# IanYeung/RealVSR

Measured on AMD Instinct MI355X. Metric: HR frames/sec (fwd+bwd) on 5-frame 180x320 LR windows, higher is better.
Workload: dtype f32 (bf16x3 GEMM); 1 GPU; EDVR-M nf64, 5-frame 180x320 LR windows, batch 8 per GPU, x4 output, VideoSRModel.optimize_parameters: fwd + LapPyr(ssim,cb) on Y + GWLoss on CbCr + bwd + Adam step; per_gpu_batch=8, global_batch=8, parallelism=sequence-dp1, gemm=bf16x3 (3-term bf16 split on v_mfma_f32_32x32x16_bf16, f32 accumulate), lf_term=ssim (restated IQA_pytorch.SSIM, parity unpinned)

## Files before the change

### include/realvsr_hip.h

```cpp
#ifndef REALVSR_HIP_H
#define REALVSR_HIP_H
#include <stddef.h>
#ifdef __cplusplus
extern "C" {
#endif

#define RVSR_OK 0
#define RVSR_ERR_UNSUPPORTED 1
#define RVSR_ERR_BAD_ARG 2
#define RVSR_ERR_LAUNCH 3
#define RVSR_ERR_WORKSPACE 4

const char* rvsr_last_error(void);

void rvsr_set_gemm_mode(int mode);
int rvsr_get_gemm_mode(void);
void rvsr_set_gemm_mode_thread(int mode);


size_t rvsr_modulated_deform_conv_forward_workspace_bytes(int channels, int channels_out);
int rvsr_modulated_deform_conv_forward(const float* input, const float* weight, const float* bias,
                                       const float* offset, const float* mask, float* output,
                                       int batch, int channels, int height, int width, int channels_out,
                                       int kernel_h, int kernel_w, int stride_h, int stride_w,
// ... 33 lines not shown
size_t rvsr_dcn_pack_weights(const float* weight, int channels, int channels_out, void* out, size_t out_bytes,
                             long long* desc, void* stream);
int rvsr_dcn_pack_forward(const float* input, const float* weight, const float* bias, const float* om,
                          float* output, int batch, int channels, int height, int width, int channels_out,
                          int stride, int pad, int dilation, int deformable_group, int act, float slope,
                          void* probe, void* workspace, size_t workspace_bytes, void* stream);
int rvsr_dcn_pack_backward(const float* input, const float* weight, const float* om, const float* grad_output,
                           const float* act_out, float act_slope, float* grad_input, float* grad_weight,
                           float* grad_bias, float* grad_om, int batch, int channels, int height, int width,
                           int channels_out, int stride, int pad, int dilation, int deformable_group,
                           const void* probe, void* workspace, size_t workspace_bytes, void* stream);
int rvsr_dcn_pack_forward_plan(const float* input, const float* weight, const float* bias, const float* om,
                               float* output, int batch, int channels, int height, int width, int channels_out,
                               int stride, int pad, int dilation, int deformable_group, int act, float slope,
                               void* probe, void* workspace, size_t workspace_bytes, long long* plan);
int rvsr_dcn_pack_backward_plan(const float* input, const float* weight, const float* om, const float* grad_output,
                                const float* act_out, float act_slope, float* grad_input, float* grad_weight,
                                float* grad_bias, float* grad_om, int batch, int channels, int height, int width,
                                int channels_out, int stride, int pad, int dilation, int deformable_group,
                                const void* probe, void* workspace, size_t workspace_bytes, long long* plan);
int rvsr_dcn_fused_takes(int batch, int channels, int height, int width, int channels_out, int kernel_h, int kernel_w, int stride_h,
                         int stride_w, int pad_h, int pad_w, int dilation_h, int dilation_w, int group, int deformable_group);
size_t rvsr_dcn_probe_samples(int batch, int deformable_group, int height_out, int width_out);
int rvsr_dcn_forward_halo(const unsigned* counters, size_t nsamples, int channels_out);

size_t rvsr_deform_conv_generic_workspace_bytes(int dtype, int channels, int height, int width, int kernel_h, int kernel_w,
                                                int stride_h, int stride_w, int pad_h, int pad_w, int dilation_h, int dilation_w);
size_t rvsr_deform_conv_generic_forward_workspace_bytes(int dtype, int channels, int height, int width, int kernel_h, int kernel_w,
                                                        int stride_h, int stride_w, int pad_h, int pad_w, int dilation_h,
                                                        int dilation_w);
int rvsr_deform_conv_generic_forward(int dtype, const void* input, const void* weight, const void* bias, const void* offset,
                                     const void* mask, void* output, int batch, int channels, int height, int width,
                                     int channels_out, int kernel_h, int kernel_w, int stride_h, int stride_w, int pad_h, int pad_w,
                                     int dilation_h, int dilation_w, int group, int deformable_group, void* workspace,
                                     size_t workspace_bytes, void* stream);
int rvsr_deform_conv_generic_backward(int dtype, const void* input, const void* weight, const void* offset, const void* mask,
                                      const void* grad_output, void* grad_input, void* grad_offset, void* grad_mask,
                                      void* grad_weight, void* grad_bias, int batch, int channels, int height, int width,
                                      int channels_out, int kernel_h, int kernel_w, int stride_h, int stride_w, int pad_h, int pad_w,
                                      int dilation_h, int dilation_w, int group, int deformable_group, void* workspace,
                                      size_t workspace_bytes, void* stream);


size_t rvsr_conv2d_forward_workspace_bytes(int C1, int C2, int Co, int ksize);
int rvsr_conv2d_forward(const float* x1, int C1, const float* x2, int C2, const float* xact, float xact_slope,
                        int in_mode, int Hs, int Ws, const float* weight, const float* bias,
                        const float* residual, float* out1, int Co1, float* out2, int Co2, int B, int ksize,
                        int stride, int w_mode, int act, float slope, int pixel_shuffle, int Hout, int Wout,
                        void* workspace, size_t workspace_bytes, void* stream);
int rvsr_conv2d_forward_plan(const float* x1, int C1, const float* x2, int C2, const float* xact, float xact_slope,
                             int in_mode, int Hs, int Ws, const float* weight, const float* bias,
                             const float* residual, float* out1, int Co1, float* out2, int Co2, int B, int ksize,
                             int stride, int w_mode, int act, float slope, int pixel_shuffle, int Hout, int Wout, int* plan);

size_t rvsr_conv2d_pack_weights(const float* weight, int C_in, int Co, int ksize, int w_mode, void* out, size_t out_bytes,
                                long long* desc, void* stream);
int rvsr_pack_weights_batched(const void* descs, int n, void* stream);

size_t rvsr_conv2d_wgrad_workspace_bytes(int C1, int C2, int Co, int B, int ksize, int stride, int Hout, int Wout);
int rvsr_conv2d_backward_weight(const float* x1, int C1, const float* x2, int C2, int Hin, int Win,
                                const float* gout, const float* gact, float gact_slope, int g_mode,
                                int Gs_h, int Gs_w, float* grad_weight, float* grad_bias, int Co, int B,
                                int ksize, int stride, int Hout, int Wout, int accumulate,
                                void* workspace, size_t workspace_bytes, void* stream);
int rvsr_conv2d_backward_weight_plan(const float* x1, int C1, const float* x2, int C2, int Hin, int Win,
                                     const float* gout, const float* gact, float gact_slope, int g_mode,
                                     int Gs_h, int Gs_w, float* grad_weight, int Co, int B, int ksize, int stride,
                                     int Hout, int Wout, int* plan);


int rvsr_upsample_bilinear_forward(const float* in, float* out, size_t planes, int H, int W, int factor,
                                   float scale, void* stream);
int rvsr_upsample_bilinear_backward(const float* gout, float* gin, size_t planes, int H, int W, int factor,
                                    float scale, void* stream);

int rvsr_maxavgpool_forward(const float* in, float* out, unsigned char* argmax, int B, int C, int H, int W,
                            void* stream);
int rvsr_maxavgpool_backward(const float* gout, const unsigned char* argmax, float* gin, int B, int C, int H,
                             int W, void* stream);

int rvsr_tsa_temporal_forward(const float* emb, const float* emb_ref, const float* aligned, float* mod,
                              float* prob, int B, int N, int C, int H, int W, int frame_major, void* stream);
int rvsr_tsa_temporal_backward(const float* gmod, const float* emb, const float* emb_ref, const float* aligned,
                               const float* prob, float* galigned, float* gemb, float* gemb_ref, int B, int N,
                               int C, int H, int W, int frame_major, void* stream);

int rvsr_tsa_output_forward(const float* fea, const float* att, const float* att_add, float* out, size_t n,
                            void* stream);
int rvsr_tsa_output_backward(const float* g, const float* fea, const float* att, float* gfea, float* gatt,
                             size_t n, void* stream);


int rvsr_pyr_down_forward(const float* in, float* out, size_t planes, int H, int W, void* stream);
int rvsr_pyr_down_backward(const float* gout, float* gin, size_t planes, int H, int W, void* stream);
int rvsr_pyr_updiff_forward(const float* cur, const float* down, float* out, size_t planes, int H, int W,
                            void* stream);
int rvsr_pyr_updiff_backward(const float* gout, float* gdown, size_t planes, int H, int W, void* stream);

size_t rvsr_charbonnier_workspace_bytes(void);
int rvsr_charbonnier_forward(const float* x, const float* y, size_t n, float eps, double scale, float* out,
                             void* workspace, void* stream);
int rvsr_charbonnier_backward(const float* x, const float* y, const float* gscalar, float scale, float eps,
                              float* gx, size_t n, void* stream);

int rvsr_gwloss_forward(const float* x1, const float* x2, size_t planes, int H, int W, float w, double scale, float* out,
                        float* fa, float* fbx, float* fby, void* workspace, void* stream);
// ... 66 lines not shown
```

### realvsr_amd/_lib.py

```python
import ctypes
import os
import subprocess

import torch

_CSRC = os.path.join(os.path.dirname(os.path.abspath(__file__)), 'csrc')
SO_PATH = os.environ.get('RVSR_SO', os.path.join(_CSRC, 'librealvsr_hip.so'))
_lib = None

c_fp = ctypes.c_void_p
c_int, c_float, c_double, c_size = ctypes.c_int, ctypes.c_float, ctypes.c_double, ctypes.c_size_t

_CONV_CALL = [c_fp, c_int, c_fp, c_int, c_fp, c_float, c_int, c_int, c_int, c_fp, c_fp, c_fp, c_fp, c_int, c_fp, c_int, c_int, c_int,
              c_int, c_int, c_int, c_float, c_int, c_int, c_int]
SIGNATURES = {
    'rvsr_last_error': (ctypes.c_char_p, []),
    'rvsr_modulated_deform_conv_forward': (c_int, [c_fp] * 6 + [c_int] * 16 + [c_fp, c_size, c_fp]),
    'rvsr_modulated_deform_conv_forward_workspace_bytes': (c_size, [c_int] * 2),
    'rvsr_modulated_deform_conv_backward_workspace_bytes': (c_size, [c_int] * 8),
    'rvsr_modulated_deform_conv_backward': (c_int, [c_fp] * 11 + [c_int] * 16 + [c_fp, c_size, c_fp]),
    'rvsr_deform_conv_workspace_bytes': (c_size, [c_int] * 11),
    'rvsr_deform_conv_forward': (c_int, [c_fp] * 4 + [c_int] * 16 + [c_fp, c_size, c_fp]),
    'rvsr_deform_conv_backward_input': (c_int, [c_fp] * 6 + [c_int] * 16 + [c_fp, c_size, c_fp]),
    'rvsr_deform_conv_backward_parameters': (c_int, [c_fp] * 4 + [c_int] * 15 + [c_float, c_int, c_fp, c_size, c_fp]),
    'rvsr_deform_conv_generic_workspace_bytes': (c_size, [c_int] * 12),
    'rvsr_deform_conv_generic_forward_workspace_bytes': (c_size, [c_int] * 12),
    'rvsr_deform_conv_generic_forward': (c_int, [c_int] + [c_fp] * 6 + [c_int] * 15 + [c_fp, c_size, c_fp]),
    'rvsr_deform_conv_generic_backward': (c_int, [c_int] + [c_fp] * 10 + [c_int] * 15 + [c_fp, c_size, c_fp]),
    'rvsr_dcn_pack_forward': (c_int, [c_fp] * 5 + [c_int] * 10 + [c_float, c_fp, c_fp, c_size, c_fp]),
    'rvsr_dcn_offset_probe': (c_int, [c_fp, c_int, c_int, c_int, c_int, c_fp, c_fp]),
    'rvsr_dcn_pack_backward': (c_int, [c_fp] * 5 + [c_float] + [c_fp] * 4 + [c_int] * 9 + [c_fp, c_fp, c_size, c_fp]),
    'rvsr_dcn_pack_forward_plan': (c_int, [c_fp] * 5 + [c_int] * 10 + [c_float, c_fp, c_fp, c_size, ctypes.POINTER(ctypes.c_longlong)]),
    'rvsr_dcn_pack_backward_plan': (c_int, [c_fp] * 5 + [c_float] + [c_fp] * 4 + [c_int] * 9 + [c_fp, c_fp, c_size,
                                                                                             ctypes.POINTER(ctypes.c_longlong)]),
    'rvsr_dcn_fused_takes': (c_int, [c_int] * 15),
    'rvsr_dcn_probe_samples': (c_size, [c_int] * 4),
    'rvsr_dcn_forward_halo': (c_int, [c_fp, c_size, c_int]),
    'rvsr_conv2d_forward': (c_int, _CONV_CALL + [c_fp, c_size, c_fp]),
    'rvsr_conv2d_forward_plan': (c_int, _CONV_CALL + [ctypes.POINTER(c_int)]),
    'rvsr_conv2d_forward_workspace_bytes': (c_size, [c_int] * 4),
    'rvsr_conv2d_pack_weights': (c_size, [c_fp, c_int, c_int, c_int, c_int, c_fp, c_size, ctypes.POINTER(ctypes.c_longlong), c_fp]),
    'rvsr_dcn_pack_weights': (c_size, [c_fp, c_int, c_int, c_fp, c_size, ctypes.POINTER(ctypes.c_longlong), c_fp]),
    'rvsr_pack_weights_batched': (c_int, [c_fp, c_int, c_fp]),
    'rvsr_set_gemm_mode': (None, [c_int]),
    'rvsr_get_gemm_mode': (c_int, []),
    'rvsr_set_gemm_mode_thread': (None, [c_int]),
    'rvsr_conv2d_wgrad_workspace_bytes': (c_size, [c_int] * 8),
    'rvsr_conv2d_backward_weight': (c_int, [c_fp, c_int, c_fp, c_int, c_int, c_int, c_fp, c_fp, c_float, c_int, c_int,
                                            c_int, c_fp, c_fp, c_int, c_int, c_int, c_int, c_int, c_int, c_int, c_fp,
                                            c_size, c_fp]),
    'rvsr_conv2d_backward_weight_plan': (c_int, [c_fp, c_int, c_fp, c_int, c_int, c_int, c_fp, c_fp, c_float, c_int, c_int, c_int, c_fp] +
                                         [c_int] * 6 + [ctypes.POINTER(c_int)]),
    'rvsr_upsample_bilinear_forward': (c_int, [c_fp, c_fp, c_size, c_int, c_int, c_int, c_float, c_fp]),
    'rvsr_upsample_bilinear_backward': (c_int, [c_fp, c_fp, c_size, c_int, c_int, c_int, c_float, c_fp]),
    'rvsr_maxavgpool_forward': (c_int, [c_fp, c_fp, c_fp, c_int, c_int, c_int, c_int, c_fp]),
    'rvsr_maxavgpool_backward': (c_int, [c_fp, c_fp, c_fp, c_int, c_int, c_int, c_int, c_fp]),
    'rvsr_tsa_temporal_forward': (c_int, [c_fp] * 5 + [c_int] * 6 + [c_fp]),
    'rvsr_tsa_temporal_backward': (c_int, [c_fp] * 8 + [c_int] * 6 + [c_fp]),
    'rvsr_tsa_output_forward': (c_int, [c_fp] * 4 + [c_size, c_fp]),
    'rvsr_tsa_output_backward': (c_int, [c_fp] * 5 + [c_size, c_fp]),
    'rvsr_pyr_down_forward': (c_int, [c_fp, c_fp, c_size, c_int, c_int, c_fp]),
    'rvsr_pyr_down_backward': (c_int, [c_fp, c_fp, c_size, c_int, c_int, c_fp]),
    'rvsr_pyr_updiff_forward': (c_int, [c_fp, c_fp, c_fp, c_size, c_int, c_int, c_fp]),
    'rvsr_pyr_updiff_backward': (c_int, [c_fp, c_fp, c_size, c_int, c_int, c_fp]),
    'rvsr_charbonnier_workspace_bytes': (c_size, []),
    'rvsr_charbonnier_forward': (c_int, [c_fp, c_fp, c_size, c_float, c_double, c_fp, c_fp, c_fp]),
    'rvsr_charbonnier_backward': (c_int, [c_fp, c_fp, c_fp, c_float, c_float, c_fp, c_size, c_fp]),
    'rvsr_gwloss_forward': (c_int, [c_fp, c_fp, c_size, c_int, c_int, c_float, c_double, c_fp, c_fp, c_fp, c_fp, c_fp, c_fp]),
    'rvsr_gwloss_backward': (c_int, [c_fp, c_fp, c_fp, c_fp, c_float, c_fp, c_size, c_int, c_int, c_fp]),
    'rvsr_ycbcr_to_bgr_u8': (c_int, [c_fp, c_fp, c_int, c_int, c_fp]),
    'rvsr_reduce_workspace_bytes': (c_size, []),
    'rvsr_pixel_loss_forward': (c_int, [c_fp, c_fp, c_size, c_int, c_float, c_double, c_fp, c_fp, c_fp]),
    'rvsr_pixel_loss_backward': (c_int, [c_fp, c_fp, c_fp, c_int, c_float, c_float, c_fp, c_size, c_fp]),
    'rvsr_ssim_forward': (c_int, [c_fp, c_fp, c_size, c_int, c_int, c_double, c_fp, c_fp, c_fp, c_fp, c_fp, c_fp]),
    'rvsr_ssim_backward': (c_int, [c_fp] * 6 + [c_float, c_fp, c_size, c_int, c_int, c_fp]),
    'rvsr_conv_gauss_forward': (c_int, [c_fp, c_fp, c_size, c_int, c_int, c_float, c_fp]),
    'rvsr_conv_gauss_backward': (c_int, [c_fp, c_fp, c_size, c_int, c_int, c_float, c_fp]),
    'rvsr_pyr_upsample_forward': (c_int, [c_fp, c_fp, c_size, c_int, c_int, c_fp]),
    'rvsr_pyr_upsample_backward': (c_int, [c_fp, c_fp, c_size, c_int, c_int, c_fp]),
    'rvsr_adam_step': (c_int, [c_fp] * 4 + [c_size] + [c_float] * 6 + [c_fp]),
    'rvsr_bcast_add_act': (c_int, [c_fp, c_fp, c_size, c_int, c_int, c_float, c_fp]),
    'rvsr_bcast_reduce_act': (c_int, [c_fp, c_fp, c_fp, c_size, c_int, c_float, c_fp]),
    'rvsr_augment_clips': (c_int, [c_fp] * 5 + [c_size] + [c_int] * 10 + [c_float, c_fp]),
    'rvsr_bn_workspace_bytes': (c_size, [c_int] * 3),
    'rvsr_bn_lrelu_forward': (c_int, [c_fp] * 9 + [c_int] * 4 + [c_float] * 3 + [c_fp, c_size, c_fp]),
    'rvsr_bn_lrelu_backward': (c_int, [c_fp] * 9 + [c_int] * 4 + [c_float, c_fp, c_size, c_fp]),
    'rvsr_gan_loss_forward': (c_int, [c_fp, c_size, c_fp, c_size, c_float, c_double, c_fp, c_fp, c_fp]),
    'rvsr_gan_loss_backward': (c_int, [c_fp, c_size, c_size, c_fp, c_fp, c_float, c_float, c_fp, c_fp, c_fp]),
    'rvsr_channel_attention_workspace_bytes': (c_size, [c_int] * 4),
    'rvsr_channel_attention_plan': (c_int, [c_int] * 4 + [c_fp] * 3 + [ctypes.POINTER(c_int)] * 2),
    'rvsr_channel_attention_forward': (c_int, [c_fp] * 10 + [c_int] * 5 + [c_float, c_fp, c_size, c_fp]),
    'rvsr_channel_attention_backward': (c_int, [c_fp] * 12 + [c_int] * 5 + [c_float, c_fp, c_size, c_fp]),
# ... 74 lines not shown
```

### realvsr_amd/csrc/conv2_kernels.hip

```cpp
#define RVSR_DEFINE_PACK
#include "conv_plan.h"

#include "bf16x3.h"

#ifdef RVSR_ABL5
constexpr int ABL5 = RVSR_ABL5;
#else
constexpr int ABL5 = 0;
#endif

#ifdef RVSR_TIMELINE
__device__ unsigned long long rvsr_dbg[512];
extern "C" int rvsr_debug_read(unsigned long long* out) { return (int)hipMemcpyFromSymbol(out, HIP_SYMBOL(rvsr_dbg), sizeof(unsigned long long) * 512); }
#define STAMP(i) do { if (blockIdx.x == 77 && tid == 0) rvsr_dbg[(i)] = __builtin_amdgcn_s_memtime(); } while (0)
#else
#define STAMP(i) do {} while (0)
#endif

template <int MT, int MODE>
__device__ __forceinline__ void conv2_epilogue(f32x16 (&acc)[MT][2], const ConvFwdParams& p, const float* bias_s, int b,
                                               int o0, int row0, int col, int hi) {
    const float neg = p.act == 0 ? 1.f : (p.act == 1 ? 0.f : p.slope);
    const bool col_ok = col < p.Wout;
    const size_t HW = (size_t)p.Hout * p.Wout;
#pragma unroll
    for (int n = 0; n < 2; ++n) {
        const int row = row0 + n;
        if (row >= p.Hout) continue;
        const size_t pix = (size_t)row * p.Wout + col;
#pragma unroll
        for (int m = 0; m < MT; ++m) {
            float resv[16];
            if (MODE == 1) {
#pragma unroll
                for (int r = 0; r < 16; ++r) {
                    const int o = o0 + m * 32 + 4 * hi + (r & 3) + 8 * (r >> 2);
                    const bool ok = col_ok && o < p.Co;
                    resv[r] = p.res[ok ? ((size_t)b * p.Co + o) * HW + pix : 0];
                }
            }
#pragma unroll
            for (int r = 0; r < 16; ++r) {
                const int ol = m * 32 + 4 * hi + (r & 3) + 8 * (r >> 2);
                const int o = o0 + ol;
                const bool ok = col_ok && o < p.Co;
                const int oc = ok ? o : 0;
                float v = acc[m][n][r] + bias_s[ol];
                v = v > 0.f ? v : v * neg;
                if (MODE == 3) {
                    const size_t idx = (((size_t)b * (p.Co >> 2) + (oc >> 2)) * (2 * p.Hout) + 2 * row + ((oc >> 1) & 1)) *
                                           (2 * p.Wout) + 2 * col + (oc & 1);
                    if (ok) p.out1[idx] = v;
                } else if (MODE == 2) {
                    const bool first = oc < p.Co1;
                    float* dst = first ? p.out1 : p.out2;
                    const size_t idx = ((size_t)b * (first ? p.Co1 : p.Co - p.Co1) + (first ? oc : oc - p.Co1)) * HW + pix;
// ... 294 lines not shown
#pragma unroll
                for (int g = 0; g < CCG; ++g) {
                    const int oc = 2 * g + hi;
                    bf16x8 ah[MT], al[MT], bh[2], bl[2];
#pragma unroll
                    for (int m = 0; m < MT; ++m) {
                        ah[m] = ws_hi[(tap * NOCT + oc) * MP + m * 32 + lo];
                        al[m] = ws_lo[(tap * NOCT + oc) * MP + m * 32 + lo];
                    }
#pragma unroll
                    for (int n = 0; n < 2; ++n) {
                        const int idx = (oc * IH + (wave * 2 + n) * STRIDE + dy) * IW + lo * STRIDE + dx;
                        bh[n] = xs_hi[idx];
                        bl[n] = xs_lo[idx];
                    }
#pragma unroll
                    for (int m = 0; m < MT; ++m)
#pragma unroll
                        for (int n = 0; n < 2; ++n) acc[m][n] = mfma_bf16(ah[m], bh[n], acc[m][n]);
#pragma unroll
                    for (int m = 0; m < MT; ++m)
#pragma unroll
                        for (int n = 0; n < 2; ++n) acc[m][n] = mfma_bf16(ah[m], bl[n], acc[m][n]);
#pragma unroll
                    for (int m = 0; m < MT; ++m)
#pragma unroll
                        for (int n = 0; n < 2; ++n) acc[m][n] = mfma_bf16(al[m], bh[n], acc[m][n]);
                }
            }
            STAMP(4 + chunk * 5);
            __syncthreads();
            STAMP(5 + chunk * 5);
        }
        if (p.ps)
            conv2_epilogue<MT, 3>(acc, p, bias_s, cb_, cmb * MP, cy0 + wave * 2, cx0 + lo, hi);
        else if (p.out2 != nullptr)
            conv2_epilogue<MT, 2>(acc, p, bias_s, cb_, cmb * MP, cy0 + wave * 2, cx0 + lo, hi);
        else if (p.res != nullptr) {
            if (p.vec4) conv2_epilogue_v4<MT, 1>(acc, p, bias_s, cb_, cmb * MP, cy0 + wave * 2, cx0, lo, hi);
            else conv2_epilogue<MT, 1>(acc, p, bias_s, cb_, cmb * MP, cy0 + wave * 2, cx0 + lo, hi);
        } else {
            if (p.vec4) conv2_epilogue_v4<MT, 0>(acc, p, bias_s, cb_, cmb * MP, cy0 + wave * 2, cx0, lo, hi);
            else conv2_epilogue<MT, 0>(acc, p, bias_s, cb_, cmb * MP, cy0 + wave * 2, cx0 + lo, hi);
        }
        STAMP(30);
        if (S + nwq < range1) {
            decode(S + nwq);
            tile_views();
            if (PF) issue_loads(0);
        }
        STAMP(31);
        __syncthreads();
    }
}

template <int MT, bool ACT_IN, int VEC, bool WIDE = false, int NT = 3>
__global__ __launch_bounds__(512, 2) void conv_fwd5_kernel(const ConvFwdParams p) {
    constexpr int KS = 3, T = 9, PAD = 1, NW = 8, TH = WIDE ? NW : 2 * NW, TW = WIDE ? 64 : 32, NTHR = NW * 64;
    constexpr int IH = TH + KS - 1, IW = TW + KS - 1;
    constexpr int MP = MT * 32, NOCT = 2, NPOS = IH * IW, NX = NOCT * NPOS;
    constexpr int WVEC = T * NOCT * MP;
    extern __shared__ __attribute__((aligned(16))) unsigned char smem_raw[];
    bf16x8* xs_base = reinterpret_cast<bf16x8*>(smem_raw);
    bf16x8* ws_base = xs_base + 2 * 2 * NX;
    float* bias_base = reinterpret_cast<float*>(ws_base + 2 * 2 * WVEC);
    bf16x8* const sink = reinterpret_cast<bf16x8*>(bias_base + 4 * MP);
    const int tid = threadIdx.x, lane = tid & 63, wave = tid >> 6, lo = lane & 31, hi = lane >> 5;
    const TView& va = p.in.a;
    const TView& vb = p.in.b;
    const int C1 = va.C, Ctot = va.C + vb.C;
    const int nchunks = (Ctot + 15) / 16;

    const unsigned nmb = (p.Co + MP - 1) / MP, nty = (p.Hout + TH - 1) / TH, ntx = (p.Wout + TW - 1) / TW;
    const unsigned items = ntx * nty * nmb * p.B;
    const unsigned xcd = blockIdx.x & 7, wq = blockIdx.x >> 3, nwq = (gridDim.x + 7 - xcd) >> 3;
    const unsigned q8 = items >> 3, r8 = items & 7;
    const unsigned range0 = xcd < r8 ? xcd * (q8 + 1) : r8 * (q8 + 1) + (xcd - r8) * q8;
    const unsigned range1 = range0 + q8 + (xcd < r8 ? 1 : 0);
    const unsigned S0 = range0 + wq;
    if (S0 >= range1) return;
    const int ntile = (int)((range1 - S0 + nwq - 1) / nwq);
    const int Q = ntile * nchunks;

    struct Tile { int x0, y0, mb, b; };
    auto tile_of = [&](int k) {
        const unsigned S = S0 + (unsigned)k * nwq;
        Tile t;
        const unsigned u = S % (ntx * nty);
        t.x0 = (int)(u % ntx) * TW;
        t.y0 = (int)(u / ntx) * TH;
        t.mb = (int)((S / (ntx * nty)) % nmb);
        t.b = (int)(S / (ntx * nty * nmb));
        return t;
    };

    constexpr int NG = TW / 4 + 2;
    __amdgpu_buffer_rsrc_t w_rs = buf_view_2g(p.wpack), xa_rs = buf_view_2g(va.p), xb_rs = buf_view_2g(va.p), act_rs = buf_view_2g(va.p);
    constexpr int NIT = VEC ? 1 : (NX + NTHR - 1) / NTHR;
    constexpr int WPARTS = NT >= 3 ? 2 : 1;
    constexpr int NWV = (WPARTS * WVEC + NTHR - 1) / NTHR;
    constexpr int NV = VEC ? 4 : 1;
    int it_oc[NIT], it_sp[NIT], it_dst[NIT];
    bool it_pos_ok[NIT];
    auto item_geom = [&](const Tile& t) {
#pragma unroll
        for (int i = 0; i < NIT; ++i) {
// ... 408 lines not shown
#define ROW(KS, STRIDE, MT, CCG) \
    if (ksize == KS && stride == STRIDE && q.mt == MT) return q.act_in ? conv_fwd2_kernel<KS, STRIDE, MT, CCG, true, 4> : conv_fwd2_kernel<KS, STRIDE, MT, CCG, false, 4>
    ROW(3, 2, 1, 1);
    ROW(3, 2, 2, 1);
    ROW(5, 1, 1, 1);
    ROW(5, 2, 1, 1);
    ROW(1, 1, 1, 2);
    ROW(1, 1, 2, 2);
#undef ROW
    return nullptr;
}

static ConvFwdKernel fwd5_kernel(const ConvFwdPlan& q) {
#define ROW(MT, VEC, WIDE, NT) \
    if (q.mt == MT && q.vec == VEC && q.wide == WIDE && q.nt == NT) return q.act_in ? conv_fwd5_kernel<MT, true, VEC, WIDE, NT> : conv_fwd5_kernel<MT, false, VEC, WIDE, NT>
    ROW(2, 1, true, 3);
    ROW(2, 1, true, 2);
    ROW(2, 1, true, 1);
    ROW(2, 1, false, 3);
    ROW(2, 1, false, 2);
    ROW(2, 1, false, 1);
    ROW(2, 2, false, 3);
    ROW(2, 2, false, 2);
    ROW(2, 2, false, 1);
    ROW(2, 3, false, 3);
    ROW(2, 3, false, 2);
    ROW(2, 3, false, 1);
    ROW(2, 0, false, 3);
    ROW(1, 0, false, 3);
    ROW(1, 1, false, 3);
    ROW(1, 2, false, 3);
    ROW(1, 3, false, 3);
#undef ROW
    if (q.mt == 2 && q.vec == 1 && q.nt == 4 && !q.act_in) return q.wide ? conv_fwd5_kernel<2, false, 1, true, 4> : conv_fwd5_kernel<2, false, 1, false, 4>;
    return nullptr;
}

int rvsr_launch_conv_fwd2(ConvFwdParams p, const ConvFwdPlan& q, int ksize, int stride, void* workspace, size_t workspace_bytes, hipStream_t st) {
    const int Ctot = p.in.a.C + p.in.b.C, T = ksize * ksize;
    int mt, ccg, nchunks, nmb;
    conv_fwd2_geom(ksize, p.Co, Ctot, mt, ccg, nchunks, nmb);
    const size_t need = rvsr_conv_fwd2_workspace_bytes(ksize, p.Co, Ctot);
    if (!workspace || workspace_bytes < need) FAIL(RVSR_ERR_WORKSPACE, "conv2d: workspace %zu B < %zu B", workspace_bytes, need);
    const bool five = q.family == CONV_FWD5;
    const ConvFwdKernel k = five ? fwd5_kernel(q) : fwd2_kernel(ksize, stride, q);
    if (!k) FAIL(RVSR_ERR_LAUNCH, "conv2d: no %s instantiation for this plan", five ? "conv_fwd5" : "conv_fwd2");
    if (!p.prepacked) {
        const size_t total = (size_t)nmb * nchunks * T * (2 * ccg) * (mt * 32);
        hipLaunchKernelGGL(pack_weights_kernel, dim3((unsigned)((total + 255) / 256)), dim3(256), 0, st, p.w, (bf16x8*)workspace, p.Co,
                           Ctot, T, mt * 32, ccg, nchunks, nmb, p.w_mode | (p.fmt ? 0x100 : 0));
    }
    p.wpack = workspace;
    p.vec4 = q.vec4;
    return rvsr_conv_launch(five ? "conv_fwd5" : "conv_fwd2", k, dim3(q.gx), five ? 512 : 256, q.lds, st, p);
}

extern "C" size_t rvsr_conv2d_pack_weights(const float* weight, int C_in, int Co, int ksize, int w_mode, void* out, size_t out_bytes,
                                           long long* desc, void* stream) {
    int mt, ccg, nchunks, nmb;
    if (ksize != 1 && ksize != 3 && ksize != 5) return 0;
    conv_fwd2_geom(ksize, Co, C_in, mt, ccg, nchunks, nmb);
    const size_t need = rvsr_conv_fwd2_workspace_bytes(ksize, Co, C_in);
    if (!weight || !out || out_bytes < need) return 0;
    if ((w_mode & 4) && !conv_f16fp8_ok(ksize, 1, mt, w_mode & 1)) return 0;
    const int fmtflag = (w_mode & 4) ? 0x100 : 0;
    const int T = ksize * ksize;
    const size_t total = (size_t)nmb * nchunks * T * (2 * ccg) * (mt * 32);
    hipLaunchKernelGGL(pack_weights_kernel, dim3((unsigned)((total + 255) / 256)), dim3(256), 0, (hipStream_t)stream, weight, (bf16x8*)out, Co,
                       C_in, T, mt * 32, ccg, nchunks, nmb, (w_mode & 1) | fmtflag);
    if (desc) {
        desc[0] = (long long)(uintptr_t)weight; desc[1] = (long long)(uintptr_t)out;
        desc[2] = Co; desc[3] = C_in; desc[4] = T; desc[5] = mt * 32; desc[6] = ccg; desc[7] = nchunks; desc[8] = nmb; desc[9] = (w_mode & 1) | fmtflag;
    }
    return need;
}
extern "C" int rvsr_pack_weights_batched(const void* descs, int n, void* stream) {
    if (n <= 0) return RVSR_OK;
    if (!descs) FAIL(RVSR_ERR_BAD_ARG, "pack_weights_batched: null table");
    static_assert(sizeof(PackDesc) == 48, "PackDesc layout is part of the C ABI (two pointers + eight ints)");
    hipLaunchKernelGGL(pack_weights_batched_kernel, dim3(16, (unsigned)n), dim3(256), 0, (hipStream_t)stream, (const PackDesc*)descs);
    hipError_t e = hipGetLastError();
    if (e != hipSuccess) FAIL(RVSR_ERR_LAUNCH, "pack_weights_batched launch: %s", hipGetErrorString(e));
    return RVSR_OK;
}

#define WG2_THREADS 512
#define WG2_GP 272
#define WG2_XP 496

typedef unsigned int u32x4 __attribute__((ext_vector_type(4)));

__device__ __forceinline__ bf16x8 as_bf16x8(u32x4 v) { return __builtin_bit_cast(bf16x8, v); }

template <int SHIFT>
__device__ __forceinline__ bf16x8 take8(u32x4 a, u32x4 b) {
    u32x4 r;
    if (SHIFT == 4) {
        r[0] = a[2]; r[1] = a[3]; r[2] = b[0]; r[3] = b[1];
    } else if (SHIFT == 3) {
        r[0] = __builtin_amdgcn_alignbit(a[2], a[1], 16);
        r[1] = __builtin_amdgcn_alignbit(a[3], a[2], 16);
        r[2] = __builtin_amdgcn_alignbit(b[0], a[3], 16);
        r[3] = __builtin_amdgcn_alignbit(b[1], b[0], 16);
    } else {
        r[0] = __builtin_amdgcn_alignbit(a[3], a[2], 16);
        r[1] = __builtin_amdgcn_alignbit(b[0], a[3], 16);
// ... 761 lines not shown
```

### realvsr_amd/csrc/conv_kernels.hip

```cpp
#include "rvsr_common.h"

#include "conv_plan.h"

template <int KS, int STRIDE, int MT, int CC>
__global__ __launch_bounds__(RVSR_WG, 2) void conv_fwd_kernel(const ConvFwdParams p) {
    constexpr int T = KS * KS, PAD = KS / 2, TH = 8, TW = 32;
    constexpr int IH = (TH - 1) * STRIDE + KS, IW = (TW - 1) * STRIDE + KS;
    constexpr int MP = MT * 32, MPP = MP + 1;
    extern __shared__ __attribute__((aligned(16))) float smem[];
    float* xs = smem;
    float* ws = smem + CC * IH * IW;
    const int tid = threadIdx.x, lane = tid & 63, wave = tid >> 6, lo = lane & 31, hi = lane >> 5;
    const int tx = blockIdx.x % p.ntx, ty = blockIdx.x / p.ntx;
    const int x0 = tx * TW, y0 = ty * TH, mb = blockIdx.y, b = blockIdx.z;
    const int Ctot = p.in.a.C + p.in.b.C;

    f32x16 acc[MT][2];
#pragma unroll
    for (int m = 0; m < MT; ++m) {
        acc[m][0] = zero16();
        acc[m][1] = zero16();
    }

    for (int c0 = 0; c0 < Ctot; c0 += CC) {
// ... 281 lines not shown
    p.Co = Co1 + Co2;
    if (pixel_shuffle && (p.Co % 4)) FAIL(RVSR_ERR_BAD_ARG, "conv2d: pixel-shuffle needs Co %% 4 == 0");
    p.B = B;
    p.Hout = Hout;
    p.Wout = Wout;
    p.w_mode = w_mode & 1;
    p.prepacked = (w_mode >> 1) & 1;
    p.fmt = (w_mode >> 2) & 1;
    p.act = act;
    p.slope = slope;
    p.ps = pixel_shuffle;
    p.ntx = (Wout + 31) / 32;
    return RVSR_OK;
}
static int conv_fwd_refuse(const ConvFwdPlan& q) {
    snprintf(rvsr_g_err, sizeof(rvsr_g_err), "%s", q.msg ? q.msg : "");
    return q.rc;
}

extern "C" int rvsr_conv2d_forward(const float* x1, int C1, const float* x2, int C2, const float* xact,
                                   float xact_slope, int in_mode, int Hs, int Ws, const float* weight,
                                   const float* bias, const float* residual, float* out1, int Co1, float* out2,
                                   int Co2, int B, int ksize, int stride, int w_mode, int act, float slope,
                                   int pixel_shuffle, int Hout, int Wout, void* workspace, size_t workspace_bytes,
                                   void* stream) {
    ConvFwdParams p;
    const int rc = conv_fwd_params(p, x1, C1, x2, C2, xact, xact_slope, in_mode, Hs, Ws, weight, bias, residual, out1, Co1, out2, Co2, B,
                                   ksize, stride, w_mode, act, slope, pixel_shuffle, Hout, Wout);
    if (rc) return rc;
    const ConvFwdPlan q = conv_fwd_plan(p, ksize, stride, rvsr_gemm_mode_now());
    if (q.rc) return conv_fwd_refuse(q);
    hipStream_t st = (hipStream_t)stream;
    switch (q.family) {
        case CONV_FWD_THIN: return rvsr_launch_conv_fwd_thin(p, q, st);
        case CONV_FWD_F32: return launch_fwd(p, q, ksize, stride, st);
        default: return rvsr_launch_conv_fwd2(p, q, ksize, stride, workspace, workspace_bytes, st);
    }
}
extern "C" int rvsr_conv2d_forward_plan(const float* x1, int C1, const float* x2, int C2, const float* xact,
                                        float xact_slope, int in_mode, int Hs, int Ws, const float* weight,
                                        const float* bias, const float* residual, float* out1, int Co1, float* out2,
                                        int Co2, int B, int ksize, int stride, int w_mode, int act, float slope,
                                        int pixel_shuffle, int Hout, int Wout, int* plan) {
    ConvFwdParams p;
    const int rc = conv_fwd_params(p, x1, C1, x2, C2, xact, xact_slope, in_mode, Hs, Ws, weight, bias, residual, out1, Co1, out2, Co2, B,
                                   ksize, stride, w_mode, act, slope, pixel_shuffle, Hout, Wout);
    if (rc) return rc;
    const ConvFwdPlan q = conv_fwd_plan(p, ksize, stride, rvsr_gemm_mode_now());
    const int row[14] = {q.family, q.mt, q.vec, q.wide, q.nt, q.act_in, q.cc, q.vec4, q.th, q.tw, (int)q.gx, (int)q.gy, (int)q.gz, (int)q.lds};
    for (int i = 0; plan && i < 14; ++i) plan[i] = row[i];
    return q.rc ? conv_fwd_refuse(q) : RVSR_OK;
}

int rvsr_g_gemm_mode = 0;
thread_local int rvsr_t_gemm_mode = -1;
extern "C" void rvsr_set_gemm_mode(int mode) { rvsr_g_gemm_mode = (mode >= 0 && mode <= 3) ? mode : 0; }
extern "C" void rvsr_set_gemm_mode_thread(int mode) { rvsr_t_gemm_mode = (mode >= 0 && mode <= 3) ? mode : -1; }
extern "C" int rvsr_get_gemm_mode() { return rvsr_gemm_mode_now(); }
extern "C" size_t rvsr_conv2d_forward_workspace_bytes(int C1, int C2, int Co, int ksize) {
    return rvsr_conv_fwd2_workspace_bytes(ksize, Co, C1 + C2);
}

extern "C" size_t rvsr_conv2d_wgrad_workspace_bytes(int C1, int C2, int Co, int B, int ksize, int stride, int Hout,
                                                    int Wout) {
    const size_t P = conv_wgrad_max_P(ksize, stride, B, Hout, Wout, Co, C1 + C2);
    return sizeof(float) * P * ((size_t)Co * (C1 + C2) * ksize * ksize + Co);
}

template <int KS, int STRIDE, int CCW>
static int launch_wgrad(const ConvWgradParams& p, int gy, int gz, hipStream_t st) {
    constexpr int IH = 3 * STRIDE + KS, IW = 31 * STRIDE + KS, CS = (IH * IW) | 1;
    return rvsr_conv_launch("conv_wgrad", conv_wgrad_kernel<KS, STRIDE, CCW>, dim3(p.P, gy, gz), RVSR_WG, sizeof(float) * (128 * 65 + CCW * CS), st, p);
}

static int conv_wgrad_params(ConvWgradParams& p, const float* x1, int C1, const float* x2, int C2, int Hin, int Win, const float* gout,
                             const float* gact, float gact_slope, int g_mode, int Gs_h, int Gs_w, float* grad_weight, int Co, int B,
                             int ksize, int stride, int Hout, int Wout) {
    if (!x1 || !gout || !grad_weight || B <= 0) FAIL(RVSR_ERR_BAD_ARG, "conv2d_backward_weight: null/empty argument");
    if ((x2 == nullptr) != (C2 == 0)) FAIL(RVSR_ERR_BAD_ARG, "conv2d_backward_weight: x2/C2 disagree");
    if (ksize != 1 && ksize != 3 && ksize != 5) FAIL(RVSR_ERR_UNSUPPORTED, "conv2d_backward_weight: kernel size %d", ksize);
    if (stride != 1 && !(stride == 2 && ksize != 1)) FAIL(RVSR_ERR_UNSUPPORTED, "conv2d_backward_weight: stride %d", stride);
    if (g_mode != 0 && g_mode != 2) FAIL(RVSR_ERR_UNSUPPORTED, "conv2d_backward_weight: gradient view mode %d", g_mode);
    make_view(p.x.a, x1, nullptr, 0.f, C1, Hin, Win, 0, 0, 0);
    make_view(p.x.b, x2, nullptr, 0.f, C2, Hin, Win, 0, 0, 0);
    if (make_view(p.g, gout, gact, gact_slope, Co, Gs_h, Gs_w, g_mode, 0, 0) || p.g.Hv != Hout || p.g.Wv != Wout)
        FAIL(RVSR_ERR_BAD_ARG, "conv2d_backward_weight: gradient view %dx%d (mode %d) vs output %dx%d", Gs_h, Gs_w, g_mode,
             Hout, Wout);
    const int pad = ksize / 2;
    if ((Hin + 2 * pad - ksize) / stride + 1 != Hout || (Win + 2 * pad - ksize) / stride + 1 != Wout)
        FAIL(RVSR_ERR_BAD_ARG, "conv2d_backward_weight: input %dx%d does not give output %dx%d", Hin, Win, Hout, Wout);
    p.part = p.bpart = nullptr;
    p.B = B;
    p.Co = Co;
    p.Hout = Hout;
    p.Wout = Wout;
    p.ntx = (Wout + 31) / 32;
    p.nty = (Hout + 3) / 4;
    p.P = 0;
    p.ring = 0;
    return RVSR_OK;
}

extern "C" int rvsr_conv2d_backward_weight_plan(const float* x1, int C1, const float* x2, int C2, int Hin, int Win,
                                                const float* gout, const float* gact, float gact_slope, int g_mode,
                                                int Gs_h, int Gs_w, float* grad_weight, int Co, int B, int ksize, int stride,
                                                int Hout, int Wout, int* plan) {
// ... 48 lines not shown
```

### realvsr_amd/csrc/conv_plan.h

```cpp
#pragma once
#include "conv_common.h"

static inline bool conv_al16(const void* a, const void* b = nullptr, const void* c = nullptr, const void* d = nullptr) {
    return ((((uintptr_t)a) | ((uintptr_t)b) | ((uintptr_t)c) | ((uintptr_t)d)) & 15) == 0;
}
static inline bool conv_span_ok(size_t H, size_t W, size_t C) { return sizeof(float) * H * W * C < ((size_t)1 << 31); }


enum ConvFwdFamily {
    CONV_FWD_THIN = 0,
    CONV_FWD5 = 1,
    CONV_FWD2 = 2,
    CONV_FWD_F32 = 3,
};

struct ConvFwdPlan {
    int rc;
    const char* msg;
    int family;
    int mt;
    int vec;
    int wide;
    int nt;
    int act_in;
    int cc;
    int vec4;
    int th, tw;
    unsigned gx, gy, gz;
    size_t lds;
};

static inline void conv_fwd2_geom(int ksize, int Co, int Ctot, int& mt, int& ccg, int& nchunks, int& nmb) {
    mt = (Co <= 32 || ksize == 5) ? 1 : 2;
    ccg = ksize == 1 ? 2 : 1;
    nchunks = (Ctot + 16 * ccg - 1) / (16 * ccg);
    nmb = (Co + mt * 32 - 1) / (mt * 32);
}
static inline bool conv_f16fp8_ok(int ksize, int stride, int mt, int w_mode) { return ksize == 3 && stride == 1 && mt == 2 && w_mode == 0; }

#define THIN_FW 136
#define THIN_FPL (10 * THIN_FW)
static inline bool conv_fwd_thin_ok(const ConvFwdParams& p, int ksize, int stride) {
    const TView& va = p.in.a;
    return ksize == 3 && stride == 1 && p.Co <= 4 && p.in.b.C == 0 && va.C % 8 == 0 && va.mode == 0 && va.act == nullptr &&
           p.out2 == nullptr && !p.ps && p.w_mode == 0 && p.Wout % 4 == 0 && va.Ws == p.Wout && va.Hs == p.Hout &&
           conv_al16(va.p, p.out1, p.res) && conv_span_ok(p.Hout, p.Wout, va.C) && va.C <= 256;
}

static inline ConvFwdPlan conv_fwd_refusal(const char* msg) {
    ConvFwdPlan r = {};
    r.rc = RVSR_ERR_UNSUPPORTED;
    r.msg = msg;
    r.family = -1;
    return r;
}

static inline ConvFwdPlan conv_fwd_plan(const ConvFwdParams& p, int ksize, int stride, int gemm_mode) {
    const TView& va = p.in.a;
    const TView& vb = p.in.b;
    const int Ctot = va.C + vb.C, T = ksize * ksize;
    if (p.act == 3 && (!p.res || ksize != 3 || stride != 1 || p.ps || p.out2 || gemm_mode == 1)) return conv_fwd_refusal(nullptr);
    ConvFwdPlan q = {};
    q.act_in = va.act != nullptr;
    q.nt = 3;
    q.th = 8;
    q.tw = 32;
    int ccg, nchunks, nmb;
    conv_fwd2_geom(ksize, p.Co, Ctot, q.mt, ccg, nchunks, nmb);
    const int ntx = (p.Wout + 31) / 32, nty8 = (p.Hout + 7) / 8;

    bool split = p.act == 3;
    const bool thin = !split && conv_fwd_thin_ok(p, ksize, stride);
    if (!split && !thin) {
        split = gemm_mode != 1 && (va.mode != 1 || ksize == 3) && (vb.C == 0 || va.C % 8 == 0);
        if (split && (ksize != 3 || stride == 2) && va.mode == 0 &&
            (!conv_span_ok(va.Hs, va.Ws, va.C > vb.C ? va.C : vb.C) || (vb.C != 0 && va.C % (16 * ccg) != 0)))
            split = false;
    }
    if (p.fmt && !(split && conv_f16fp8_ok(ksize, stride, q.mt, p.w_mode)))
        return conv_fwd_refusal("conv2d: the f16 + fp8 format (w_mode | 4) is for forward 3x3 / stride-1 convs with more than 32 output channels");

    if (thin) {
        q.family = CONV_FWD_THIN;
        q.mt = 1;
        q.tw = 128;
        q.gx = (unsigned)p.B * nty8 * ((p.Wout + 127) / 128);
        q.gy = q.gz = 1;
        q.lds = sizeof(float) * (8 * THIN_FPL + (size_t)va.C * 36);
        return q;
    }
    if (!split) {
        q.family = CONV_FWD_F32;
        q.mt = p.Co <= 32 ? 1 : (p.Co <= 64 ? 2 : 4);
        const int wide_m = q.mt == 4;
        q.cc = ksize == 1 ? 32 : ksize == 3 ? (stride == 1 ? (wide_m ? 8 : 16) : (wide_m ? 4 : 8)) : (stride == 1 ? (wide_m ? 4 : 8) : 4);
        const int IH = 7 * stride + ksize, IW = 31 * stride + ksize;
        q.lds = sizeof(float) * ((size_t)q.cc * IH * IW + (size_t)T * q.cc * (q.mt * 32 + 1));
        q.gx = (unsigned)(ntx * nty8);
        q.gy = (unsigned)((p.Co + q.mt * 32 - 1) / (q.mt * 32));
        q.gz = (unsigned)p.B;
        return q;
    }
    q.vec4 = (p.Wout % 4 == 0) && conv_al16(p.out1, p.res) && !p.ps && p.out2 == nullptr && conv_span_ok(p.Hout, p.Wout, p.Co);
    q.cc = ccg;
    q.gy = q.gz = 1;
    long items = (long)nmb * p.B;
    if (ksize != 3 || stride != 1) {
        q.family = CONV_FWD2;
        const int IH = 7 * stride + ksize, IW = 31 * stride + ksize;
        q.lds = (size_t)16 * (2 * (2 * ccg) * IH * IW + 2 * T * (2 * ccg) * (q.mt * 32)) + sizeof(float) * q.mt * 32;
        items *= (long)ntx * nty8;
        const int slots = 256 * (q.lds > 80 * 1024 ? 1 : 2);
        q.gx = (unsigned)(items < slots ? items : slots);
        return q;
    }
    q.family = CONV_FWD5;
    const bool al = conv_al16(va.p, va.act, vb.p);
    if (va.mode == 0 && va.Ws % 4 == 0 && va.Wv == va.Ws && al && conv_span_ok(va.Hs, va.Ws, va.C > vb.C ? va.C : vb.C) &&
        (vb.C == 0 || va.C % 16 == 0))
        q.vec = 1;
    else if (va.mode == 2 && vb.C == 0 && va.C % 16 == 0 && va.Wv % 4 == 0 && va.Ws == 2 * va.Wv && va.Hs == 2 * va.Hv && al &&
             conv_span_ok(va.Hs, va.Ws, va.C >> 2))
        q.vec = 2;
    else if (va.mode == 1 && vb.C == 0 && va.Wv % 4 == 0 && va.Wv == 2 * va.Ws && va.Hv <= 2 * va.Hs && va.Ws % 2 == 0 && al &&
             conv_span_ok(va.Hs, va.Ws, va.C))
        q.vec = 3;
    if (p.fmt && (q.vec != 1 || q.act_in))
        return conv_fwd_refusal("conv2d: the f16 + fp8 format needs a plain 16-byte-aligned input view with W % 4 == 0 and no act' tensor");
    const long px_n = (long)((p.Hout + 15) / 16 * 16) * ((p.Wout + 31) / 32 * 32), px_w = (long)((p.Hout + 7) / 8 * 8) * ((p.Wout + 63) / 64 * 64);
    q.wide = q.mt == 2 && q.vec == 1 && q.vec4 && px_w <= px_n;
    if (p.act == 3 && !q.wide) return conv_fwd_refusal(nullptr);
    if (p.fmt) q.nt = 4;
    else if (q.mt == 2 && q.vec != 0) q.nt = gemm_mode == 2 ? 2 : (gemm_mode == 3 ? 1 : 3);
    q.th = q.wide ? 8 : 16;
    q.tw = q.wide ? 64 : 32;
    const int NX = q.wide ? 2 * 10 * 66 : 2 * 18 * 34, WVEC = 9 * 2 * q.mt * 32;
    q.lds = (size_t)16 * (2 * 2 * NX + 2 * 2 * WVEC) + sizeof(float) * 4 * q.mt * 32 + 16;
    items *= (long)((p.Wout + q.tw - 1) / q.tw) * ((p.Hout + q.th - 1) / q.th);
    q.gx = (unsigned)(items < 256 ? items : 256);
    return q;
}

enum ConvWgradFamily {
    CONV_WGRAD_THIN = 0,
    CONV_WGRAD2,
    CONV_WGRAD5,
    CONV_WGRAD_F32_5,
    CONV_WGRAD_1X1S,
    CONV_WGRAD_1X1,
    CONV_WGRAD_F32_3S1,
    CONV_WGRAD_S2,
    CONV_WGRAD_F32_3S2,
    CONV_WGRAD_F32_1,
    CONV_WGRAD_FAMILIES
};
struct ConvWgradPlan {
    int family, P, gy, gz;
};

static inline bool conv_wgrad_can(int family, int ksize, int stride, int Co) {
    switch (family) {
        case CONV_WGRAD_THIN: return ksize == 3 && stride == 1 && Co <= 4;
        case CONV_WGRAD2: case CONV_WGRAD_F32_3S1: return ksize == 3 && stride == 1;
        case CONV_WGRAD5: case CONV_WGRAD_F32_5: return ksize == 5;
        case CONV_WGRAD_S2: case CONV_WGRAD_F32_3S2: return ksize == 3 && stride == 2;
        default: return ksize == 1;
// ... 79 lines not shown
```

Before: 83.78 HR frames/s.

## Add streaming persistent 1x1 conv forward kernel with XCD-aware tile scheduling

Adds a new persistent kernel for 1x1 stride-1 convolutions. It runs one workgroup per CU, and the work is split into contiguous ranges per XCD. Each block streams 512-pixel tiles through double-buffered LDS with register prefetch, holds activations resident across output-channel blocks when there are two input chunks, and fuses bias, activation and residual into a vectorized epilogue. It is meant to beat the generic conv_fwd2 path on large 1x1 layers by overlapping global loads with bf16x3 MFMA work. The cost is a new, complex kernel with its own occupancy and scheduling assumptions, plus a variant query API.

New measurement: 84.16 HR frames/s (median of 6 runs). No clear change (+0.4%).

```diff
diff --git a/include/realvsr_hip.h b/include/realvsr_hip.h
--- a/include/realvsr_hip.h
+++ b/include/realvsr_hip.h
@@ -109,6 +109,10 @@
                              int in_mode, int Hs, int Ws, const float* weight, const float* bias,
                              const float* residual, float* out1, int Co1, float* out2, int Co2, int B, int ksize,
                              int stride, int w_mode, int act, float slope, int pixel_shuffle, int Hout, int Wout, int* plan);
+int rvsr_conv2d_forward_variant(const float* x1, int C1, const float* x2, int C2, const float* xact, float xact_slope,
+                                int in_mode, int Hs, int Ws, const float* weight, const float* bias,
+                                const float* residual, float* out1, int Co1, float* out2, int Co2, int B, int ksize,
+                                int stride, int w_mode, int act, float slope, int pixel_shuffle, int Hout, int Wout, int* variant);
 
 size_t rvsr_conv2d_pack_weights(const float* weight, int C_in, int Co, int ksize, int w_mode, void* out, size_t out_bytes,
                                 long long* desc, void* stream);
diff --git a/realvsr_amd/_lib.py b/realvsr_amd/_lib.py
--- a/realvsr_amd/_lib.py
+++ b/realvsr_amd/_lib.py
@@ -38,6 +38,7 @@
     'rvsr_dcn_forward_halo': (c_int, [c_fp, c_size, c_int]),
     'rvsr_conv2d_forward': (c_int, _CONV_CALL + [c_fp, c_size, c_fp]),
     'rvsr_conv2d_forward_plan': (c_int, _CONV_CALL + [ctypes.POINTER(c_int)]),
+    'rvsr_conv2d_forward_variant': (c_int, _CONV_CALL + [ctypes.POINTER(c_int)]),
     'rvsr_conv2d_forward_workspace_bytes': (c_size, [c_int] * 4),
     'rvsr_conv2d_pack_weights': (c_size, [c_fp, c_int, c_int, c_int, c_int, c_fp, c_size, ctypes.POINTER(ctypes.c_longlong), c_fp]),
     'rvsr_dcn_pack_weights': (c_size, [c_fp, c_int, c_int, c_fp, c_size, ctypes.POINTER(ctypes.c_longlong), c_fp]),
diff --git a/realvsr_amd/csrc/conv2_kernels.hip b/realvsr_amd/csrc/conv2_kernels.hip
--- a/realvsr_amd/csrc/conv2_kernels.hip
+++ b/realvsr_amd/csrc/conv2_kernels.hip
@@ -2,6 +2,7 @@
 #include "conv_plan.h"
 
 #include "bf16x3.h"
+#include <type_traits>
 
 #ifdef RVSR_ABL5
 constexpr int ABL5 = RVSR_ABL5;
@@ -402,6 +403,229 @@
         STAMP(31);
         __syncthreads();
     }
+}
+
+template <int MODE>
+__device__ __forceinline__ void conv2s_epilogue(f32x16 (&acc)[2][2], const ConvFwdParams& p, const float* bias_s, int b, int o0, int pxw,
+                                                int lo, int hi) {
+    const float neg = p.act == 0 ? 1.f : (p.act == 1 ? 0.f : p.slope);
+    const int j = lo & 3;
+    const unsigned HW = (unsigned)(p.Hout * p.Wout), HW4 = 4u * HW;
+    const __amdgpu_buffer_rsrc_t out_rs = buf_view_2g(p.out1 + (size_t)b * p.Co * HW);
+    const __amdgpu_buffer_rsrc_t res_rs = buf_view_2g(MODE == 1 ? p.res + (size_t)b * p.Co * HW : p.out1);
+#pragma unroll
+    for (int n = 0; n < 2; ++n) {
+        const unsigned px = (unsigned)(pxw + 32 * n + (lo & ~3));
+        const bool px_ok = px < HW;
+        const unsigned lane_off = 4u * ((unsigned)(4 * hi + j) * HW + px);
+#pragma unroll
+        for (int m = 0; m < 2; ++m) {
+#pragma unroll
+            for (int rp = 0; rp < 4; rp += 2) {
+                float4 resv[2];
+                unsigned off[2];
+#pragma unroll
+                for (int r2 = 0; r2 < 2; ++r2) {
+                    const int ob = o0 + m * 32 + 8 * (rp + r2);
+                    off[r2] = (px_ok && ob + 4 * hi + j < p.Co ? lane_off : 0x80000000u) + (ob < p.Co ? (unsigned)ob * HW4 : 0u);
+                    if (MODE == 1) {
+                        typedef float f32x4v __attribute__((ext_vector_type(4)));
+                        const f32x4v q = __builtin_bit_cast(f32x4v, __builtin_amdgcn_raw_buffer_load_b128(res_rs, (int)off[r2], 0, 0));
+                        resv[r2] = make_float4(q.x, q.y, q.z, q.w);
+                    }
+                }
+#pragma unroll
+                for (int r2 = 0; r2 < 2; ++r2) {
+                    const int rg = rp + r2;
+                    float r0 = acc[m][n][4 * rg + 0], r1 = acc[m][n][4 * rg + 1], r2_ = acc[m][n][4 * rg + 2], r3 = acc[m][n][4 * rg + 3];
+                    quad_transpose4(r0, r1, r2_, r3, lo);
+                    const float bb = bias_s[m * 32 + 8 * rg + 4 * hi + j];
+                    float4 v = make_float4(r0 + bb, r1 + bb, r2_ + bb, r3 + bb);
+                    v.x = v.x > 0.f ? v.x : v.x * neg; v.y = v.y > 0.f ? v.y : v.y * neg;
+                    v.z = v.z > 0.f ? v.z : v.z * neg; v.w = v.w > 0.f ? v.w : v.w * neg;
+                    if (MODE == 1) { v.x += resv[r2].x; v.y += resv[r2].y; v.z += resv[r2].z; v.w += resv[r2].w; }
+                    buf_store4(out_rs, off[r2], 0u, v);
+                }
+            }
+        }
+    }
+}
+
+template <bool ACT_IN, bool RESIDENT>
+__global__ __launch_bounds__(F2S_THREADS, 1) void conv_fwd2s_kernel(const ConvFwdParams p) {
+    constexpr int XROW = F2S_XROW, XBUF = 2 * 4 * XROW, WBUF = 2 * 4 * 64;
+    constexpr unsigned OOB = 0x80000000u;
+    extern __shared__ __attribute__((aligned(16))) unsigned char smem_raw[];
+    bf16x8* xs = reinterpret_cast<bf16x8*>(smem_raw);
+    bf16x8* ws = xs + 2 * XBUF;
+    float* bias_s = reinterpret_cast<float*>(ws + 2 * WBUF);
+    const int tid = threadIdx.x, lane = tid & 63, wave = tid >> 6, lo = lane & 31, hi = lane >> 5;
+    const TView& va = p.in.a;
+    const TView& vb = p.in.b;
+    const int C1 = va.C, Ctot = va.C + vb.C;
+    const int nchunks = (Ctot + 31) / 32, nmb = (p.Co + 63) / 64;
+    const int HW = p.Hout * p.Wout;
+    const unsigned hw4 = 4u * (unsigned)HW;
+    const unsigned tpi = (unsigned)(HW + F2S_TP - 1) / F2S_TP;
+
+    const unsigned items = tpi * p.B;
+    const unsigned xcd = blockIdx.x & 7, wq = blockIdx.x >> 3, nwq = (gridDim.x + 7 - xcd) >> 3;
+    const unsigned q8 = items >> 3, r8 = items & 7;
+    const unsigned range0 = xcd < r8 ? xcd * (q8 + 1) : r8 * (q8 + 1) + (xcd - r8) * q8;
+    const unsigned range1 = range0 + q8 + (xcd < r8 ? 1 : 0);
+    const unsigned S0 = range0 + wq;
+    if (S0 >= range1) return;
+    const int ntile = (int)((range1 - S0 + nwq - 1) / nwq);
+    constexpr bool resident = RESIDENT;
+    const int Q = ntile * nmb * nchunks;
+
+    for (int i = tid; i < nmb * 64; i += F2S_THREADS) bias_s[i] = (p.bias != nullptr && i < p.Co) ? p.bias[i] : 0.f;
+
+    typedef float f32x4v __attribute__((ext_vector_type(4)));
+    f32x4v xr[2][8];
+    f32x4v ar[ACT_IN ? 8 : 1];
+    bf16x8 wr[2];
+    const int ocx = __builtin_amdgcn_readfirstlane(tid >> 7), gx4 = tid & 127;
+    const __amdgpu_buffer_rsrc_t w_rs = buf_view_2g(p.wpack);
+
+    struct Cursor { int k, c, m; };
+    Cursor xcur = {0, 0, 0}, acur = {0, 0, 0};
+    int wm = 0, wc = 0;
+    auto advance = [&](Cursor& u) {
+        if (++u.c == nchunks) {
+            u.c = 0;
+            if (resident || ++u.m == nmb) { u.m = 0; ++u.k; }
+        }
+    };
+    auto issue8 = [&](const Cursor& u, f32x4v (&dst)[8], bool act) {
+        const bool valid = u.k < ntile;
+        const unsigned S = valid ? S0 + (unsigned)u.k * nwq : S0;
+        const unsigned b = S / tpi, t0 = (S - b * tpi) * (F2S_TP / 4);
+        const int c0 = u.c * 32;
+        const bool second = c0 >= C1;
+        const int Cb = second ? vb.C : va.C, cl0 = (second ? c0 - C1 : c0) + 8 * ocx;
+        const __amdgpu_buffer_rsrc_t rs = buf_view_2g((act ? va.act : (second ? vb.p : va.p)) + (size_t)b * Cb * HW);
+        const unsigned quad = t0 + (unsigned)gx4;
+        const unsigned vo = valid && 4u * quad < (unsigned)HW ? 16u * quad : OOB;
+#pragma unroll
+        for (int j = 0; j < 8; ++j) {
+            const unsigned vo_j = cl0 + j < Cb ? vo : OOB;
+            const unsigned so = (unsigned)(cl0 + j) * hw4;
+            dst[j] = __builtin_bit_cast(f32x4v, __builtin_amdgcn_raw_buffer_load_b128(rs, (int)vo_j, (int)so, 0));
+        }
+    };
+    auto issue_x = [&](auto par) {
+        constexpr int PAR = decltype(par)::value;
+        issue8(xcur, xr[PAR], false);
+        advance(xcur);
+    };
+    auto issue_a = [&]() {
+        if (ACT_IN) {
+            issue8(acur, reinterpret_cast<f32x4v (&)[8]>(ar), true);
+            advance(acur);
+        }
+    };
+    auto issue_w = [&](auto par) {
+        constexpr int PAR = decltype(par)::value;
+        const unsigned so = (unsigned)(wm * nchunks + wc) * (WBUF * 16u);
+        wr[PAR] = __builtin_bit_cast(bf16x8, __builtin_amdgcn_raw_buffer_load_b128(w_rs, tid * 16, (int)so, 0));
+        if (++wc == nchunks) {
+            wc = 0;
+            if (++wm == nmb) wm = 0;
+        }
+    };
+    auto commit_x = [&](auto par) {
+        constexpr int PAR = decltype(par)::value;
+        bf16x8* dst = xs + PAR * XBUF + ocx * XROW + gx4;
+#pragma unroll
+        for (int e = 0; e < 4; ++e) {
+            float v[8];
+#pragma unroll
+            for (int j = 0; j < 8; ++j) v[j] = ACT_IN ? xr[PAR][j][e] * (ar[ACT_IN ? j : 0][e] > 0.f ? 1.f : va.slope) : xr[PAR][j][e];
+            bf16x8 h8, l8;
+            split8(v, h8, l8);
+            dst[e * 132] = h8;
+            dst[4 * XROW + e * 132] = l8;
+        }
+    };
+
+    f32x16 acc[2][2];
+    int ck = 0, cm = 0, cc = 0;
+    unsigned cb_ = S0 / tpi, cpx0 = (S0 - cb_ * tpi) * F2S_TP;
+    auto step = [&](auto par) {
+        constexpr int PAR = decltype(par)::value;
+        const bool xload = !resident || cm == 0;
+        if (xload) commit_x(par);
+        ws[PAR * WBUF + tid] = wr[PAR];
+        __syncthreads();
+        issue_w(par);
+        __builtin_amdgcn_sched_barrier(0);
+        if (xload) {
+            issue_a();
+            issue_x(par);
+        }
+        __builtin_amdgcn_sched_barrier(0);
+        if (cc == 0) {
+#pragma unroll
+            for (int m = 0; m < 2; ++m) {
+                acc[m][0] = zero16();
+                acc[m][1] = zero16();
+            }
+        }
+        const bf16x8* xb = xs + PAR * XBUF;
+        const bf16x8* wb = ws + PAR * WBUF;
+#pragma unroll
+        for (int g = 0; g < 2; ++g) {
+            const int oc = 2 * g + hi;
+            bf16x8 ah[2], al[2];
+#pragma unroll
+            for (int m = 0; m < 2; ++m) {
+                ah[m] = wb[oc * 64 + m * 32 + lo];
+                al[m] = wb[4 * 64 + oc * 64 + m * 32 + lo];
+            }
+#pragma unroll
+            for (int n = 0; n < 2; ++n) {
+                const int idx = oc * XROW + (lo & 3) * 132 + ((wave * 64 + n * 32 + lo) >> 2);
+                const bf16x8 bh = xb[idx], bl = xb[4 * XROW + idx];
+#pragma unroll
+                for (int m = 0; m < 2; ++m) acc[m][n] = mfma_bf16(ah[m], bh, acc[m][n]);
+#pragma unroll
+                for (int m = 0; m < 2; ++m) acc[m][n] = mfma_bf16(ah[m], bl, acc[m][n]);
+#pragma unroll
+                for (int m = 0; m < 2; ++m) acc[m][n] = mfma_bf16(al[m], bh, acc[m][n]);
+            }
+        }
+        if (++cc == nchunks) {
+            cc = 0;
+            if (p.res != nullptr) conv2s_epilogue<1>(acc, p, bias_s + cm * 64, (int)cb_, cm * 64, (int)cpx0 + wave * 64, lo, hi);
+            else conv2s_epilogue<0>(acc, p, bias_s + cm * 64, (int)cb_, cm * 64, (int)cpx0 + wave * 64, lo, hi);
+            if (++cm == nmb) {
+                cm = 0;
+                ++ck;
+                const unsigned S = S0 + (unsigned)ck * nwq;
+                cb_ = S / tpi;
+                cpx0 = (S - cb_ * tpi) * F2S_TP;
+            }
+        }
+    };
+
+    const std::integral_constant<int, 0> P0;
+    const std::integral_constant<int, 1> P1;
+    issue_w(P0);
+    __builtin_amdgcn_sched_barrier(0);
+    issue_x(P0);
+    __builtin_amdgcn_sched_barrier(0);
+    issue_w(P1);
+    __builtin_amdgcn_sched_barrier(0);
+    issue_a();
+    issue_x(P1);
+    __builtin_amdgcn_sched_barrier(0);
+    int q = 0;
+    for (; q + 1 < Q; q += 2) {
+        step(P0);
+        step(P1);
+    }
+    if (q < Q) step(P0);
 }
 
 template <int MT, bool ACT_IN, int VEC, bool WIDE = false, int NT = 3>
@@ -916,6 +1140,12 @@
     }
     p.wpack = workspace;
     p.vec4 = q.vec4;
+    if (!five && q.stream) {
+        const bool resident = nchunks == 2 && nmb > 1;
+        const ConvFwdKernel ks = q.act_in ? (resident ? conv_fwd2s_kernel<true, true> : conv_fwd2s_kernel<true, false>)
+                                          : (resident ? conv_fwd2s_kernel<false, true> : conv_fwd2s_kernel<false, false>);
+        return rvsr_conv_launch("conv_fwd2s", ks, dim3(q.gx), F2S_THREADS, q.lds, st, p);
+    }
     return rvsr_conv_launch(five ? "conv_fwd5" : "conv_fwd2", k, dim3(q.gx), five ? 512 : 256, q.lds, st, p);
 }
 
diff --git a/realvsr_amd/csrc/conv_kernels.hip b/realvsr_amd/csrc/conv_kernels.hip
--- a/realvsr_amd/csrc/conv_kernels.hip
+++ b/realvsr_amd/csrc/conv_kernels.hip
@@ -357,6 +357,20 @@
     return q.rc ? conv_fwd_refuse(q) : RVSR_OK;
 }
 
+extern "C" int rvsr_conv2d_forward_variant(const float* x1, int C1, const float* x2, int C2, const float* xact,
+                                           float xact_slope, int in_mode, int Hs, int Ws, const float* weight,
+                                           const float* bias, const float* residual, float* out1, int Co1, float* out2,
+                                           int Co2, int B, int ksize, int stride, int w_mode, int act, float slope,
+                                           int pixel_shuffle, int Hout, int Wout, int* variant) {
+    ConvFwdParams p;
+    const int rc = conv_fwd_params(p, x1, C1, x2, C2, xact, xact_slope, in_mode, Hs, Ws, weight, bias, residual, out1, Co1, out2, Co2, B,
+                                   ksize, stride, w_mode, act, slope, pixel_shuffle, Hout, Wout);
+    if (rc) return rc;
+    const ConvFwdPlan q = conv_fwd_plan(p, ksize, stride, rvsr_gemm_mode_now());
+    if (variant) *variant = q.rc ? 0 : q.stream;
+    return q.rc ? conv_fwd_refuse(q) : RVSR_OK;
+}
+
 int rvsr_g_gemm_mode = 0;
 thread_local int rvsr_t_gemm_mode = -1;
 extern "C" void rvsr_set_gemm_mode(int mode) { rvsr_g_gemm_mode = (mode >= 0 && mode <= 3) ? mode : 0; }
diff --git a/realvsr_amd/csrc/conv_plan.h b/realvsr_amd/csrc/conv_plan.h
--- a/realvsr_amd/csrc/conv_plan.h
+++ b/realvsr_amd/csrc/conv_plan.h
@@ -28,7 +28,22 @@
     int th, tw;
     unsigned gx, gy, gz;
     size_t lds;
-};
+    int stream;
+};
+
+#define F2S_THREADS 512
+#define F2S_TP 512
+#define F2S_XROW (4 * 132)
+#define F2S_CUS 256
+static inline size_t conv_fwd2s_lds(int Co) { return (size_t)16 * (2 * 2 * 4 * F2S_XROW + 2 * 2 * 4 * 64) + sizeof(float) * 64 * ((Co + 63) / 64); }
+static inline bool conv_fwd2s_takes(const ConvFwdParams& p, const ConvFwdPlan& q, int ksize, int stride) {
+    const TView& va = p.in.a;
+    const TView& vb = p.in.b;
+    if (ksize != 1 || stride != 1 || q.mt != 2 || va.mode != 0 || !q.vec4 || p.act == 3) return false;
+    if (va.Ws % 4 != 0 || !conv_al16(va.p, va.act, vb.p) || (vb.C != 0 && va.C % 64 != 0)) return false;
+    const long tiles = (long)p.B * (((long)p.Hout * p.Wout + F2S_TP - 1) / F2S_TP);
+    return tiles >= F2S_CUS;
+}
 
 static inline void conv_fwd2_geom(int ksize, int Co, int Ctot, int& mt, int& ccg, int& nchunks, int& nmb) {
     mt = (Co <= 32 || ksize == 5) ? 1 : 2;
@@ -112,6 +127,13 @@
         items *= (long)ntx * nty8;
         const int slots = 256 * (q.lds > 80 * 1024 ? 1 : 2);
         q.gx = (unsigned)(items < slots ? items : slots);
+        if (conv_fwd2s_takes(p, q, ksize, stride)) {
+            q.stream = 1;
+            q.th = 1;
+            q.tw = F2S_TP;
+            q.gx = F2S_CUS;
+            q.lds = conv_fwd2s_lds(p.Co);
+        }
         return q;
     }
     q.family = CONV_FWD5;
```
